# montyhall/bot7

Measured on AMD Instinct MI355X. Metric: EI candidates scored/sec at N=2048,d=32, higher is better.
Workload: dtype f64

## Files before the change

### bot7_amd/csrc/covar.hip

```cpp
#include "b7_internal.h"
#include "gemm_f64.h"
#include "ksx_exp.h"

namespace {

__constant__ double exp2_tab_dev[128];

__global__ void __launch_bounds__(64) prep_obs_kernel(const double *__restrict__ xobs, const double *ls, double *w,
                                                      double *zsc, double *zsh, int N, int Npad, int d, int dpad) {
  extern __shared__ __align__(16) double psm[];
  {
    const int64_t b = blockIdx.y;
    ls += b * d;
    w += b * dpad;
    zsc += b * (int64_t)Npad * dpad;
    zsh += b * Npad;
  }
  const int tld = dpad + 1, lane = threadIdx.x, row0 = blockIdx.x * 64;
  double *tile = psm, *wl = psm + 64 * tld;
  for (int k = lane; k < dpad; k += 64) {
    const double wk = (k < d) ? 1.0 / ls[k] : 0.0;
    wl[k] = wk;
    if (blockIdx.x == 0) w[k] = wk;
  }
  int nrows = N - row0;
  nrows = nrows < 0 ? 0 : (nrows > 64 ? 64 : nrows);
  const double *src = xobs + (int64_t)row0 * d;
#pragma unroll 8
  for (int e = lane; e < nrows * d; e += 64) {
    const int r = e / d, k = e - r * d;
    tile[r * tld + k] = src[e];
  }
  __syncthreads();
  double s = 0.0;
#pragma unroll 8
  for (int k = 0; k < dpad; ++k) {
    const double z = (lane < nrows && k < d) ? tile[lane * tld + k] : 0.0;
    const double wk = wl[k];
    tile[lane * tld + k] = z * wk;
    s += (z * z) * wk;
  }
  if (row0 + lane < Npad) zsh[row0 + lane] = (lane < nrows) ? 0.5 * s : 1e300;
  __syncthreads();
  double *dst = zsc + (int64_t)row0 * dpad;
#pragma unroll 8
  for (int e = lane; e < 64 * dpad; e += 64) {
    const int r = e / dpad, k = e - r * dpad;
    if (row0 + r < Npad) dst[e] = tile[r * tld + k];
  }
}

__device__ __forceinline__ void pair_pack(double a, double b, d2_t &out) {
  const int alo = __double2loint(a), ahi = __double2hiint(a), blo = __double2loint(b), bhi = __double2hiint(b);
  int o0l, o0h, o1l, o1h;
  asm volatile(
      "s_mov_b32 vcc_lo, 0x55555555\n\t"
      "s_mov_b32 vcc_hi, 0x55555555\n\t"
      "s_nop 0\n\t"
      "v_cndmask_b32_dpp %0, %6, %4, vcc quad_perm:[1,0,3,2] row_mask:0xf bank_mask:0xf\n\t"
      "v_cndmask_b32_dpp %1, %7, %5, vcc quad_perm:[1,0,3,2] row_mask:0xf bank_mask:0xf\n\t"
      "s_not_b64 vcc, vcc\n\t"
      "v_cndmask_b32_dpp %2, %4, %6, vcc quad_perm:[1,0,3,2] row_mask:0xf bank_mask:0xf\n\t"
      "v_cndmask_b32_dpp %3, %5, %7, vcc quad_perm:[1,0,3,2] row_mask:0xf bank_mask:0xf"
      : "=&v"(o0l), "=&v"(o0h), "=&v"(o1l), "=&v"(o1h)
      : "v"(alo), "v"(ahi), "v"(blo), "v"(bhi)
      : "vcc", "scc");
  out[0] = __hiloint2double(o0h, o0l);
  out[1] = __hiloint2double(o1h, o1l);
}

constexpr int KQ = 64;
__host__ __device__ constexpr int ksx_slab(int dpad) { return dpad >= 48 ? 32 : 64; }

using KBatch = KBatchDesc;
template <int DPAD, int KERN>
__global__ void __launch_bounds__(256)
    ksx_kernel(const double *__restrict__ xq, int64_t row0, int64_t Mtotal, int d, int dpad_rt, const double *w,
               const double *zsc, const double *zsh, const double *__restrict__ alpha, double amp, double meanc, int Npad,
               double *out, double *__restrict__ mu, KBatch kb) {
  extern __shared__ __align__(16) double sm[];
  if (kb.amp) {
    const int64_t bz = blockIdx.z;
    w += bz * kb.s_w;
    zsc += bz * kb.s_zsc;
    zsh += bz * kb.s_zsh;
    out += bz * kb.s_out;
    amp = kb.amp[bz];
    if (kb.mean) {
      alpha += bz * kb.s_alpha;
      mu += bz * kb.s_mu;
      meanc = kb.mean[bz];
    }
  }
  constexpr int KO = ksx_slab(DPAD);
  constexpr int TPR = 256 / KO;
  constexpr int dpad = DPAD, NCH = (DPAD / 2 + TPR - 1) / TPR, KSTEPS = DPAD / 4;
  constexpr int stride = DPAD + 1;
  (void)dpad_rt;
  constexpr int R0 = (KQ * stride > 2 * KO * stride) ? KQ * stride : 2 * KO * stride;
  double *sq = sm;
  double *so = sm;
  double *sh = sm + R0;
  double *sal = sh + 2 * KO;
  double *shq = sal + 2 * KO;
  double *stab = shq + KQ;
  const int tid = threadIdx.x, lane = tid & 63, wave = tid >> 6;
  const int lr = lane & 15, lq = lane >> 4;
  const int64_t qbase = row0 + (int64_t)blockIdx.x * KQ;
  const int srow = tid / TPR, sq4 = tid % TPR;
  const int qrow = tid >> 2, qq4 = tid & 3;
  constexpr int half = DPAD >> 1;

  if (tid < 128) stab[tid] = amp * exp2_tab_dev[tid];
  {
    int64_t g = qbase + qrow;
    if (g > Mtotal - 1) g = Mtotal - 1;
    for (int k = qq4; k < dpad; k += 4) sq[qrow * stride + k] = (k < d) ? xq[g * d + k] : 0.0;
  }
  const int nslab_total = Npad / KO;
  const int nslab = nslab_total / gridDim.y;
  const int slab0 = blockIdx.y * nslab;

  d2_t pre[NCH];
  double pre_h = 0.0, pre_a = 0.0;
  auto load_slab = [&](int s) {
    const double *src = zsc + (int64_t)(s * KO + srow) * dpad;
#pragma unroll
    for (int i = 0; i < NCH; ++i) {
      const int kc = i * TPR + sq4;
      if (kc < half) pre[i] = *reinterpret_cast<const d2_t *>(src + 2 * kc);
    }
    if (tid < KO) {
      pre_h = zsh[s * KO + tid];
      pre_a = alpha ? alpha[s * KO + tid] : 0.0;
    }
  };
  auto store_slab = [&](int buf) {
    double *dst = so + buf * KO * stride + srow * stride;
#pragma unroll
    for (int i = 0; i < NCH; ++i) {
      const int kc = i * TPR + sq4;
      if (kc < half) {
        dst[2 * kc] = pre[i][0];
        dst[2 * kc + 1] = pre[i][1];
      }
    }
    if (tid < KO) {
      sh[buf * KO + tid] = pre_h;
      sal[buf * KO + tid] = pre_a;
    }
  };

  load_slab(slab0);
  __syncthreads();
  if (tid < KQ) {
    double s = 0.0;
    for (int k = 0; k < dpad; ++k) {
      double x = sq[tid * stride + k];
      s += (x * x) * w[k];
    }
    shq[tid] = 0.5 * s;
  }
  double qf[KSTEPS];
#pragma unroll
  for (int k4 = 0; k4 < KSTEPS; ++k4) qf[k4] = sq[(wave * 16 + lr) * stride + lq + 4 * k4];
  __syncthreads();
  store_slab(0);
  __syncthreads();

  double hq[4], macc[4] = {0.0, 0.0, 0.0, 0.0};
#pragma unroll
  for (int r = 0; r < 4; ++r) hq[r] = shq[wave * 16 + lq + 4 * r];
  const bool odd = lane & 1;
  double *orow = out + ((int64_t)blockIdx.x * KQ + wave * 16 + lq + (odd ? 4 : 0)) * Npad + (lr & ~1);

  int cur = 0;
  for (int s = 0; s < nslab; ++s) {
    const bool more = (s + 1) < nslab;
    if (more) load_slab(slab0 + s + 1);
    const double *sob = so + cur * KO * stride;
    const int o0 = (slab0 + s) * KO;
#pragma unroll
    for (int t = 0; t < KO / 16; ++t) {
      const double *ob = sob + (t * 16 + lr) * stride + lq;
      d4_t c = {0.0, 0.0, 0.0, 0.0};
      {
        double bf[KSTEPS];
#pragma unroll
        for (int k4 = 0; k4 < KSTEPS; ++k4) bf[k4] = ob[4 * k4];
#if B7_KSX_ABLATE & 8
        c = mfma_f64(qf[0], bf[0], c);
#else
#pragma unroll
        for (int k4 = 0; k4 < KSTEPS; ++k4) c = mfma_f64(qf[k4], bf[k4], c);
#endif
      }
      const double hk = sh[cur * KO + t * 16 + lr];
      const double al = sal[cur * KO + t * 16 + lr];
      double kv[4], arg[4];
#pragma unroll
      for (int r = 0; r < 4; ++r) arg[r] = (c[r] - hq[r]) - hk;
#if B7_KSX_ABLATE & 4
#pragma unroll
      for (int r = 0; r < 4; ++r) kv[r] = arg[r];
#else
      cov_nonpos4<KERN>(arg, stab, kv);
#endif
#pragma unroll
      for (int r = 0; r < 4; ++r) macc[r] = __builtin_fma(kv[r], al, macc[r]);
      d2_t v01, v23;
      pair_pack(kv[0], kv[1], v01);
      pair_pack(kv[2], kv[3], v23);
      {
        double *p = orow + o0 + t * 16;
#if B7_KSX_ABLATE & 1
        if (v01[0] == 1.2345e-300) {
#endif
#if B7_KSX_ABLATE & 16
        double *pi = out + ((int64_t)blockIdx.x * KQ + wave * 16 + 4 * t + (lane >> 5)) * Npad + o0 + (lane & 31) * 2;
        *reinterpret_cast<d2_t *>(pi) = v01;
        *reinterpret_cast<d2_t *>(pi + (int64_t)2 * Npad) = v23;
#elif B7_KSX_ABLATE & 32
        __builtin_nontemporal_store(v01, reinterpret_cast<d2_t *>(p));
        __builtin_nontemporal_store(v23, reinterpret_cast<d2_t *>(p + (int64_t)8 * Npad));
#else
        *reinterpret_cast<d2_t *>(p) = v01;
        *reinterpret_cast<d2_t *>(p + (int64_t)8 * Npad) = v23;
#endif
#if B7_KSX_ABLATE & 1
        }
#endif
      }
    }
    if (more) store_slab(cur ^ 1);
    __syncthreads();
    cur ^= 1;
  }

  if (mu) {
#pragma unroll
    for (int r = 0; r < 4; ++r) {
      double v = macc[r];
      v += __shfl_xor(v, 1);
      v += __shfl_xor(v, 2);
      v += __shfl_xor(v, 4);
      v += __shfl_xor(v, 8);
      const int64_t g = qbase + wave * 16 + lq + 4 * r;
      if (lr == 0 && g < Mtotal) mu[g] = meanc + v;
    }
  }
}

__global__ void __launch_bounds__(256)
    kxx_fix_kernel(double *K, int N, int Npad, double diag_add, const double *diag_arr, int64_t sK) {
  if (diag_arr) {
    K += (int64_t)blockIdx.y * sK;
    diag_add = diag_arr[blockIdx.y];
  }
  int64_t e = (int64_t)blockIdx.x * blockDim.x + threadIdx.x;
  if (e >= (int64_t)Npad * Npad) return;
  int i = (int)(e / Npad), j = (int)(e - (int64_t)i * Npad);
  if (i >= N || j >= N)
    K[e] = (i == j) ? 1.0 : 0.0;
  else if (i == j)
    K[e] += diag_add;
}

size_t ksx_lds_bytes(int dpad) {
  const int KO = ksx_slab(dpad);
  const size_t r0 = (size_t)(KQ > 2 * KO ? KQ : 2 * KO) * (dpad + 1);
  size_t bytes = sizeof(double) * (r0 + 4 * KO + KQ + 128);
#if B7_KSX_ABLATE & 128
  const size_t per_cu = 160 * 1024, fit = per_cu / bytes;
  if (fit > 1) bytes = per_cu / (fit - 1) - 512;
#endif
  return bytes;
}

int ensure_exp_table(b7_ctx *c) {
  static bool done[64] = {false};
  if (c->device < 64 && done[c->device]) return B7_OK;
  B7_HIP(c, hipMemcpyToSymbol(HIP_SYMBOL(exp2_tab_dev), b7_exp2_tab, sizeof(b7_exp2_tab)));
  if (c->device < 64) done[c->device] = true;
  return B7_OK;
}

template <int DPAD, int KERN>
int ksx_launch(b7_ctx *c, dim3 grid, const double *xq, int64_t row0, int64_t Mtotal, int d, const ObsSet &o,
               const double *alpha, double meanc, double *out, double *mu) {
  const size_t lds = ksx_lds_bytes(DPAD);
  auto kern = ksx_kernel<DPAD, KERN>;
  B7_TRY(ensure_exp_table(c));
  B7_HIP(c, hipFuncSetAttribute(reinterpret_cast<const void *>(kern), hipFuncAttributeMaxDynamicSharedMemorySize,
                                (int)lds));
  hipLaunchKernelGGL(kern, grid, dim3(256), lds, c->stream, xq, row0, Mtotal, d, c->dpad, o.w ? o.w : (const double *)c->w.p,
                     o.zsc, o.zsh, alpha, c->amp, meanc, o.npad, out, mu, o.batch);
  B7_HIP(c, hipGetLastError());
  return B7_OK;
}

template <int KERN>
int ksx_dispatch_k(b7_ctx *c, dim3 grid, const double *xq, int64_t row0, int64_t Mtotal, int d, const ObsSet &o,
                   const double *alpha, double meanc, double *out, double *mu) {
  switch (c->dpad) {
    case 4: return ksx_launch<4, KERN>(c, grid, xq, row0, Mtotal, d, o, alpha, meanc, out, mu);
    case 8: return ksx_launch<8, KERN>(c, grid, xq, row0, Mtotal, d, o, alpha, meanc, out, mu);
    case 16: return ksx_launch<16, KERN>(c, grid, xq, row0, Mtotal, d, o, alpha, meanc, out, mu);
    case 32: return ksx_launch<32, KERN>(c, grid, xq, row0, Mtotal, d, o, alpha, meanc, out, mu);
    case 48: return ksx_launch<48, KERN>(c, grid, xq, row0, Mtotal, d, o, alpha, meanc, out, mu);
    case 64: return ksx_launch<64, KERN>(c, grid, xq, row0, Mtotal, d, o, alpha, meanc, out, mu);
    case 96: return ksx_launch<96, KERN>(c, grid, xq, row0, Mtotal, d, o, alpha, meanc, out, mu);
    default: return b7_fail(c, B7_ERR_UNSUPPORTED, "covariance kernel: dpad %d is not a built class", c->dpad);
  }
}

int ksx_dispatch(b7_ctx *c, dim3 grid, const double *xq, int64_t row0, int64_t Mtotal, int d, const ObsSet &o,
                 const double *alpha, double meanc, double *out, double *mu) {
  if (c->kernel == B7_KERNEL_MATERN52) return ksx_dispatch_k<B7_KERNEL_MATERN52>(c, grid, xq, row0, Mtotal, d, o, alpha, meanc, out, mu);
  return ksx_dispatch_k<B7_KERNEL_ARDSE>(c, grid, xq, row0, Mtotal, d, o, alpha, meanc, out, mu);
}

}

int launch_prep_obs(b7_ctx *c, const double *xobs, const double *ls_dev, int N, int d) {
  PhaseScope ps(c, "prep");
  const size_t lds = sizeof(double) * (64 * (size_t)(c->dpad + 1) + c->dpad);
  hipLaunchKernelGGL(prep_obs_kernel, dim3((c->Npad + 63) / 64), dim3(64), lds, c->stream, xobs, ls_dev,
                     (double *)c->w.p, (double *)c->zsc.p, (double *)c->zss.p, N, c->Npad, d, c->dpad);
  B7_HIP(c, hipGetLastError());
  return B7_OK;
}

int launch_prep_obs_aux(b7_ctx *c, const double *xobs, const double *ls_dev, int N, int npad, double *zsc,
                        double *zsh) {
  const size_t lds = sizeof(double) * (64 * (size_t)(c->dpad + 1) + c->dpad);
  hipLaunchKernelGGL(prep_obs_kernel, dim3((npad + 63) / 64), dim3(64), lds, c->stream, xobs, ls_dev, (double *)c->w.p,
                     zsc, zsh, N, npad, c->dfit, c->dpad);
  B7_HIP(c, hipGetLastError());
  return B7_OK;
}

int launch_k_generic(b7_ctx *c, const double *xq, int64_t rows, int64_t Mtotal, const ObsSet &o, double *out) {
  if (rows % KQ || o.npad % 64) return b7_fail(c, B7_ERR_INVALID, "k_generic: extents not multiples of 64");
  return ksx_dispatch(c, dim3((unsigned)(rows / KQ), 1), xq, 0, Mtotal, c->dfit, o, nullptr, 0.0, out, nullptr);
}

int launch_ksx(b7_ctx *c, const double *xq, int64_t row0, int64_t rows, int64_t Mtotal, int d, double *ks,
               double *mu, int ycols) {
  PhaseScope ps(c, "ksx");
  if (rows % KQ) return b7_fail(c, B7_ERR_INVALID, "ksx: rows %lld not a multiple of %d", (long long)rows, KQ);
  if (ycols != 1) mu = nullptr;
  const ObsSet o{(const double *)c->zsc.p, (const double *)c->zss.p, c->Npad};
  return ksx_dispatch(c, dim3((unsigned)(rows / KQ), 1), xq, row0, Mtotal, d, o,
                      mu ? (const double *)c->alpha.p : nullptr, c->mean, ks, mu);
}

int launch_kxx(b7_ctx *c, double diag_add) {
  PhaseScope ps(c, "kxx");
  const int Npad = c->Npad;
  int ny = 1;
  while (ny < 16 && (Npad / 64) % (ny * 2) == 0 && (Npad / KQ) * ny < 2 * c->cus) ny *= 2;
  const ObsSet o{(const double *)c->zsc.p, (const double *)c->zss.p, Npad};
  B7_TRY(ksx_dispatch(c, dim3(Npad / KQ, ny), (const double *)c->xobs.p, 0, c->N, c->dfit, o, nullptr, 0.0,
                      (double *)c->K.p, nullptr));
  int64_t total = (int64_t)Npad * Npad;
  hipLaunchKernelGGL(kxx_fix_kernel, dim3((unsigned)((total + 255) / 256)), dim3(256), 0, c->stream, (double *)c->K.p,
                     c->N, Npad, diag_add, (const double *)nullptr, (int64_t)0);
  B7_HIP(c, hipGetLastError());
  return B7_OK;
}

int launch_ksx_batch(b7_ctx *c, int S, const double *xq, int64_t rows, int64_t Mtotal, const double *w, const double *zsc,
                     const double *zss, const double *amp_dev, const double *mean_dev, const double *alpha, double *ks,
                     int64_t s_out, double *mu, int64_t s_mu) {
  PhaseScope ps(c, "ksx");
  if (rows % KQ) return b7_fail(c, B7_ERR_INVALID, "ksx: rows %lld not a multiple of %d", (long long)rows, KQ);
  ObsSet o{zsc, zss, c->Npad};
  o.w = w;
  o.batch.s_w = c->dpad;
  o.batch.s_zsc = (int64_t)c->Npad * c->dpad;
  o.batch.s_zsh = c->Npad;
  o.batch.s_out = s_out;
  o.batch.amp = amp_dev;
  o.batch.s_alpha = c->Npad;
  o.batch.s_mu = s_mu;
  o.batch.mean = mean_dev;
  return ksx_dispatch(c, dim3((unsigned)(rows / KQ), 1, S), xq, 0, Mtotal, c->dfit, o, alpha, 0.0, ks, mu);
}

int launch_kxx_batch(b7_ctx *c, int B, const double *ls_dev, const double *amp_dev, const double *noise_dev, double *w,
                     double *zsc, double *zss, double *K) {
  PhaseScope ps(c, "kxx");
  const int Npad = c->Npad, d = c->dfit, dpad = c->dpad;
  const size_t lds = sizeof(double) * (64 * (size_t)(dpad + 1) + dpad);
  hipLaunchKernelGGL(prep_obs_kernel, dim3((Npad + 63) / 64, B), dim3(64), lds, c->stream, (const double *)c->xobs.p, ls_dev,
                     w, zsc, zss, c->N, Npad, d, dpad);
  ObsSet o{zsc, zss, Npad};
  o.w = w;
  o.batch.s_w = dpad;
  o.batch.s_zsc = (int64_t)Npad * dpad;
  o.batch.s_zsh = Npad;
  o.batch.s_out = (int64_t)Npad * Npad;
  o.batch.amp = amp_dev;
  int ny = 1;
  while (ny < 16 && (Npad / 64) % (ny * 2) == 0 && (Npad / KQ) * ny * B < 2 * c->cus) ny *= 2;
  B7_TRY(ksx_dispatch(c, dim3(Npad / KQ, ny, B), (const double *)c->xobs.p, 0, c->N, d, o, nullptr, 0.0, K, nullptr));
  const int64_t total = (int64_t)Npad * Npad;
  hipLaunchKernelGGL(kxx_fix_kernel, dim3((unsigned)((total + 255) / 256), B), dim3(256), 0, c->stream, K, c->N, Npad, 0.0,
                     noise_dev, total);
  B7_HIP(c, hipGetLastError());
  return B7_OK;
}
```

Baseline: 16.12 million.

## Transpose MFMA operands in ksx kernel to drop DPP pair-pack and set waves_per_eu

Swaps the MFMA operand order so each lane's accumulator holds training-point columns for a single query row. The row permutation of observation tiles makes each lane's four outputs land as two contiguous d2 pairs, so the inline-asm DPP pair_pack shuffle is no longer needed. The hq and alpha/h lookups become vector LDS loads. The mean reduction now folds across lanes 16 and 32 instead of four xor shuffles per register. It also adds an amdgpu_waves_per_eu attribute chosen per DPAD and kernel, which trades register budget for occupancy.

```diff
diff --git a/bot7_amd/csrc/covar.hip b/bot7_amd/csrc/covar.hip
--- a/bot7_amd/csrc/covar.hip
+++ b/bot7_amd/csrc/covar.hip
@@ -50,31 +50,44 @@
   }
 }
 
-__device__ __forceinline__ void pair_pack(double a, double b, d2_t &out) {
-  const int alo = __double2loint(a), ahi = __double2hiint(a), blo = __double2loint(b), bhi = __double2hiint(b);
-  int o0l, o0h, o1l, o1h;
-  asm volatile(
-      "s_mov_b32 vcc_lo, 0x55555555\n\t"
-      "s_mov_b32 vcc_hi, 0x55555555\n\t"
-      "s_nop 0\n\t"
-      "v_cndmask_b32_dpp %0, %6, %4, vcc quad_perm:[1,0,3,2] row_mask:0xf bank_mask:0xf\n\t"
-      "v_cndmask_b32_dpp %1, %7, %5, vcc quad_perm:[1,0,3,2] row_mask:0xf bank_mask:0xf\n\t"
-      "s_not_b64 vcc, vcc\n\t"
-      "v_cndmask_b32_dpp %2, %4, %6, vcc quad_perm:[1,0,3,2] row_mask:0xf bank_mask:0xf\n\t"
-      "v_cndmask_b32_dpp %3, %5, %7, vcc quad_perm:[1,0,3,2] row_mask:0xf bank_mask:0xf"
-      : "=&v"(o0l), "=&v"(o0h), "=&v"(o1l), "=&v"(o1h)
-      : "v"(alo), "v"(ahi), "v"(blo), "v"(bhi)
-      : "vcc", "scc");
-  out[0] = __hiloint2double(o0h, o0l);
-  out[1] = __hiloint2double(o1h, o1l);
-}
-
 constexpr int KQ = 64;
 __host__ __device__ constexpr int ksx_slab(int dpad) { return dpad >= 48 ? 32 : 64; }
 
+__device__ __forceinline__ constexpr int ksx_tile_row(int g, int r) {
+#if B7_KSX_ABLATE & 64
+  return 8 * g + r;
+#elif B7_KSX_ABLATE & 16
+  return 4 * g + r;
+#else
+  return 8 * (r >> 1) + 2 * g + (r & 1);
+#endif
+}
+__device__ __forceinline__ constexpr int ksx_tile_base(int t) { return (B7_KSX_ABLATE & 64) ? 16 * (t & ~1) : 16 * t; }
+__device__ __forceinline__ constexpr int ksx_tile_shift(int t) { return (B7_KSX_ABLATE & 64) ? 4 * (t & 1) : 0; }
+
+__device__ __forceinline__ double ksx_mean_fold(const double (&macc)[4]) {
+#if B7_KSX_ABLATE & (16 | 64)
+  double v = (macc[0] + macc[1]) + (macc[2] + macc[3]);
+  v += __shfl_xor(v, 16);
+  v += __shfl_xor(v, 32);
+  return v;
+#else
+  double lo = macc[0] + macc[1], hi = macc[2] + macc[3];
+  lo += __shfl_xor(lo, 16);
+  hi += __shfl_xor(hi, 16);
+  lo += __shfl_xor(lo, 32);
+  hi += __shfl_xor(hi, 32);
+  return lo + hi;
+#endif
+}
+
+__host__ __device__ constexpr int ksx_waves_per_simd(int dpad, int kern) {
+  return kern == B7_KERNEL_ARDSE ? (dpad == 48 ? 4 : 3) : (dpad <= 64 ? 3 : 2);
+}
+
 using KBatch = KBatchDesc;
 template <int DPAD, int KERN>
-__global__ void __launch_bounds__(256)
+__global__ void __launch_bounds__(256) __attribute__((amdgpu_waves_per_eu(ksx_waves_per_simd(DPAD, KERN), 4)))
     ksx_kernel(const double *__restrict__ xq, int64_t row0, int64_t Mtotal, int d, int dpad_rt, const double *w,
                const double *zsc, const double *zsh, const double *__restrict__ alpha, double amp, double meanc, int Npad,
                double *out, double *__restrict__ mu, KBatch kb) {
@@ -168,11 +181,11 @@
   store_slab(0);
   __syncthreads();
 
-  double hq[4], macc[4] = {0.0, 0.0, 0.0, 0.0};
-#pragma unroll
-  for (int r = 0; r < 4; ++r) hq[r] = shq[wave * 16 + lq + 4 * r];
-  const bool odd = lane & 1;
-  double *orow = out + ((int64_t)blockIdx.x * KQ + wave * 16 + lq + (odd ? 4 : 0)) * Npad + (lr & ~1);
+  const double hq = shq[wave * 16 + lr];
+  double macc[4] = {0.0, 0.0, 0.0, 0.0};
+  const int arow = ksx_tile_row(lr & 3, lr >> 2);
+  const int j01 = ksx_tile_row(lq, 0), j23 = ksx_tile_row(lq, 2);
+  double *orow = out + ((int64_t)blockIdx.x * KQ + wave * 16 + lr) * Npad;
 
   int cur = 0;
   for (int s = 0; s < nslab; ++s) {
@@ -182,50 +195,48 @@
     const int o0 = (slab0 + s) * KO;
 #pragma unroll
     for (int t = 0; t < KO / 16; ++t) {
-      const double *ob = sob + (t * 16 + lr) * stride + lq;
+      const int tb = ksx_tile_base(t);
+      const double *ob = sob + (tb + arow + ksx_tile_shift(t)) * stride + lq;
       d4_t c = {0.0, 0.0, 0.0, 0.0};
       {
-        double bf[KSTEPS];
-#pragma unroll
-        for (int k4 = 0; k4 < KSTEPS; ++k4) bf[k4] = ob[4 * k4];
+        double af[KSTEPS];
+#pragma unroll
+        for (int k4 = 0; k4 < KSTEPS; ++k4) af[k4] = ob[4 * k4];
 #if B7_KSX_ABLATE & 8
-        c = mfma_f64(qf[0], bf[0], c);
+        c = mfma_f64(af[0], qf[0], c);
 #else
 #pragma unroll
-        for (int k4 = 0; k4 < KSTEPS; ++k4) c = mfma_f64(qf[k4], bf[k4], c);
+        for (int k4 = 0; k4 < KSTEPS; ++k4) c = mfma_f64(af[k4], qf[k4], c);
 #endif
       }
-      const double hk = sh[cur * KO + t * 16 + lr];
-      const double al = sal[cur * KO + t * 16 + lr];
+      const int c01 = tb + j01 + ksx_tile_shift(t), c23 = tb + j23 + ksx_tile_shift(t);
+      const d2_t h01 = *reinterpret_cast<const d2_t *>(sh + cur * KO + c01), h23 = *reinterpret_cast<const d2_t *>(sh + cur * KO + c23);
+      const double hk[4] = {h01[0], h01[1], h23[0], h23[1]};
       double kv[4], arg[4];
 #pragma unroll
-      for (int r = 0; r < 4; ++r) arg[r] = (c[r] - hq[r]) - hk;
+      for (int r = 0; r < 4; ++r) arg[r] = (c[r] - hq) - hk[r];
 #if B7_KSX_ABLATE & 4
 #pragma unroll
       for (int r = 0; r < 4; ++r) kv[r] = arg[r];
 #else
       cov_nonpos4<KERN>(arg, stab, kv);
 #endif
-#pragma unroll
-      for (int r = 0; r < 4; ++r) macc[r] = __builtin_fma(kv[r], al, macc[r]);
-      d2_t v01, v23;
-      pair_pack(kv[0], kv[1], v01);
-      pair_pack(kv[2], kv[3], v23);
+      const d2_t a01 = *reinterpret_cast<const d2_t *>(sal + cur * KO + c01), a23 = *reinterpret_cast<const d2_t *>(sal + cur * KO + c23);
+      const double al[4] = {a01[0], a01[1], a23[0], a23[1]};
+#pragma unroll
+      for (int r = 0; r < 4; ++r) macc[r] = __builtin_fma(kv[r], al[r], macc[r]);
       {
-        double *p = orow + o0 + t * 16;
+        const d2_t v01 = {kv[0], kv[1]}, v23 = {kv[2], kv[3]};
+        double *p = orow + o0;
 #if B7_KSX_ABLATE & 1
         if (v01[0] == 1.2345e-300) {
 #endif
-#if B7_KSX_ABLATE & 16
-        double *pi = out + ((int64_t)blockIdx.x * KQ + wave * 16 + 4 * t + (lane >> 5)) * Npad + o0 + (lane & 31) * 2;
-        *reinterpret_cast<d2_t *>(pi) = v01;
-        *reinterpret_cast<d2_t *>(pi + (int64_t)2 * Npad) = v23;
-#elif B7_KSX_ABLATE & 32
-        __builtin_nontemporal_store(v01, reinterpret_cast<d2_t *>(p));
-        __builtin_nontemporal_store(v23, reinterpret_cast<d2_t *>(p + (int64_t)8 * Npad));
+#if B7_KSX_ABLATE & 32
+        __builtin_nontemporal_store(v01, reinterpret_cast<d2_t *>(p + c01));
+        __builtin_nontemporal_store(v23, reinterpret_cast<d2_t *>(p + c23));
 #else
-        *reinterpret_cast<d2_t *>(p) = v01;
-        *reinterpret_cast<d2_t *>(p + (int64_t)8 * Npad) = v23;
+        *reinterpret_cast<d2_t *>(p + c01) = v01;
+        *reinterpret_cast<d2_t *>(p + c23) = v23;
 #endif
 #if B7_KSX_ABLATE & 1
         }
@@ -238,16 +249,9 @@
   }
 
   if (mu) {
-#pragma unroll
-    for (int r = 0; r < 4; ++r) {
-      double v = macc[r];
-      v += __shfl_xor(v, 1);
-      v += __shfl_xor(v, 2);
-      v += __shfl_xor(v, 4);
-      v += __shfl_xor(v, 8);
-      const int64_t g = qbase + wave * 16 + lq + 4 * r;
-      if (lr == 0 && g < Mtotal) mu[g] = meanc + v;
-    }
+    const double v = ksx_mean_fold(macc);
+    const int64_t g = qbase + wave * 16 + lr;
+    if (lq == 0 && g < Mtotal) mu[g] = meanc + v;
   }
 }
 
```

New measurement: 16.11 million. About the same (-0.0%).
